# xxayt/MGSV

Measured on AMD Instinct MI355X. Metric: video-music pairs/s fwd+bwd at B=64 (full training step); sub-objects: retrieval sim-matrix GB/s, eval forward pairs/s, higher is better.
Workload: dtype bf16; 1 GPU; BASELINE.json configs[2]: B=64/GPU, T_v=30, T_a=512, D=512, train mode (dropout on), f32 master weights + Adam, f32 gradient accumulation; global_batch=64, launch=tape

## Files before the change

### include/made_hip.h

```cpp
#ifndef MADE_HIP_H
#define MADE_HIP_H

#include <stdint.h>

#ifdef __cplusplus
extern "C" {
#endif

#define MADE_ABI_VERSION 8

enum MadeDtype { MADE_F32 = 0, MADE_BF16 = 1 };

enum MadeAct {
    MADE_ACT_NONE = 0,
    MADE_ACT_RELU = 1,
    MADE_ACT_GELU = 2,
    MADE_ACT_QUICKGELU = 3,
    MADE_ACT_SIGMOID = 4
};

enum MadeGate {
    MADE_GATE_NONE = 0,
    MADE_GATE_RELU_OUT = 1,
    MADE_GATE_GELU_Z = 2,
// ... 438 lines not shown
                        float* save_mean, float* save_rstd, void* y, int32_t y_dtype, int64_t ldy,
                        int64_t B, int64_t T, int64_t F, void* stream);
int made_posbn_relu_bwd(const void* x, int32_t x_dtype, int64_t ldx, const void* y, int32_t y_dtype, int64_t ldy,
                        const void* dy, int32_t dy_dtype, int64_t lddy, const float* weight, const float* save_mean,
                        const float* save_rstd, int32_t batch_stats, void* dx, int32_t dx_dtype, int64_t lddx,
                        float* dweight, float* dbias, int64_t B, int64_t T, int64_t F, void* stream);

int made_set_criterion_bwd(const float* pred_logits, const float* pred_spans, const float* targets,
                           const int64_t* pred_idx, const int64_t* tgt_idx, const int32_t* count,
                           const float* proj_queries, const float* vid_sum, const float* empty_weight,
                           int64_t n_layers, int64_t B, int64_t Q, int64_t G, int64_t Dc, int32_t fg_label,
                           float temperature, const float* weights, const float* upstream,
                           float* d_logits, float* d_spans, int64_t ld_out, int32_t through_sigmoid,
                           float* d_proj_queries, float* d_vid_sum, void* stream);

#define MADE_ADAM_MAX_GROUPS 4
#define MADE_ADAM_NORM_BLOCKS 1024
typedef struct MadeAdamGroup { int64_t begin, end; float lr; float max_norm; } MadeAdamGroup;
int made_adam_step(float* param, const float* grad, float* exp_avg, float* exp_avg_sq, int64_t n,
                   const MadeAdamGroup* groups, int32_t n_groups, float beta1, float beta2, float eps, int64_t step,
                   float grad_scale, float* norm_ws, void* stream);

typedef struct MadeAdamDeviceState { int64_t step; float lr[MADE_ADAM_MAX_GROUPS]; float bc1, bc2_sqrt; } MadeAdamDeviceState;
int made_adam_step_device(float* param, const float* grad, float* exp_avg, float* exp_avg_sq, int64_t n,
                          const MadeAdamGroup* groups, int32_t n_groups, float beta1, float beta2, float eps,
                          MadeAdamDeviceState* state_device, int32_t advance_state, float grad_scale, float* norm_ws, void* stream);

typedef struct MadeRepackDesc {
    const float* src; void* w; void* wt;
    int64_t rows, cols, wt_ld, tile_begin;
// ... 85 lines not shown
```

### mgsv_amd/_lib.py

```python
from __future__ import annotations

import ctypes as C
import os

_HERE = os.path.dirname(os.path.abspath(__file__))


def variant_env(name: str, default: str = "") -> str:
    if os.environ.get("MADE_DEBUG_VARIANTS", "0") in ("", "0"):
        return default
    return os.environ.get(name, default)


LIB_PATH = os.environ.get("MADE_LIB_PATH") or os.path.join(_HERE, "libmade_hip.so")
ABI_VERSION = 8

F32, BF16 = 0, 1
ACT_NONE, ACT_RELU, ACT_GELU, ACT_QUICKGELU, ACT_SIGMOID = 0, 1, 2, 3, 4
GATE_NONE, GATE_RELU_OUT, GATE_GELU_Z, GATE_QUICKGELU_Z, GATE_SIGMOID_OUT = 0, 1, 2, 3, 4

vp, i64, i32, f32 = C.c_void_p, C.c_int64, C.c_int32, C.c_float


class MadeDropout(C.Structure):
# ... 214 lines not shown
    "made_pool_bwd": (C.c_int, [vp, vp, vp, vp, i32, i64, i64, vp, i32, i64, i64, vp, i32, i64, i64, i64, i64, i64, f32, vp]),
    "made_l2norm_bwd": (C.c_int, [vp, i32, i64, vp, i64, i64, vp, i64, i32, vp, i32, i64, i64, i64, f32, vp]),
    "made_clip_loss_bwd": (C.c_int, [vp, i64, i64, vp, f32, vp, vp, vp, vp, i32, vp, vp, vp]),
    "made_xpool_tail_bwd": (C.c_int, [vp, i32, i64, vp, vp, vp, i64, vp, i64, vp, i32, i64, vp, C.POINTER(MadeDropout),
                                      vp, vp, vp, i64, vp, i64, f32, i64, i64, i64, f32, vp]),
    "made_softmax_bwd": (C.c_int, [vp, i64, vp, i64, vp, i64, vp, f32, C.POINTER(MadeDropout), vp, vp, vp, i32, i64, i64,
                                   i64, i64, i64, i64, i64, vp]),
    "made_head_bias": (C.c_int, [vp, i32, i64, vp, vp, i64, i64, i64, vp]),
    "made_head_bias_bwd": (C.c_int, [vp, i32, i64, vp, vp, vp, vp, i64, i64, i64, vp]),
    "made_add3": (C.c_int, [vp, i32, vp, i32, vp, i32, vp, i32, i64, i64, vp]),
    "made_colsum": (C.c_int, [vp, i32, i64, i64, i64, vp, vp]),
    "made_posbn_relu_fwd": (C.c_int, [vp, i32, i64, vp, vp, vp, vp, C.c_float, C.c_float, i32, vp, vp, vp, i32, i64, i64, i64, i64, vp]),
    "made_posbn_relu_bwd": (C.c_int, [vp, i32, i64, vp, i32, i64, vp, i32, i64, vp, vp, vp, i32, vp, i32, i64, vp, vp, i64, i64, i64, vp]),
    "made_set_criterion_bwd": (C.c_int, [vp, vp, vp, vp, vp, vp, vp, vp, vp, i64, i64, i64, i64, i64, i32, f32, vp, vp,
                                         vp, vp, i64, i32, vp, vp, vp]),
    "made_adam_step": (C.c_int, [vp, vp, vp, vp, i64, C.POINTER(MadeAdamGroup), i32, f32, f32, f32, i64, f32, vp, vp]),
    "made_adam_step_device": (C.c_int, [vp, vp, vp, vp, i64, C.POINTER(MadeAdamGroup), i32, f32, f32, f32, vp, i32, f32, vp, vp]),
    "made_repack": (C.c_int, [vp, i32, i64, vp]),
    "made_row_groups": (C.c_int, [vp, i64, vp, vp]),
    "made_row_index": (C.c_int, [vp, i64, vp, vp, vp]),
    "made_linear_variant": (C.c_int, [C.POINTER(MadeLinearArgs)]),
    "made_row_affine": (C.c_int, [vp, i32, i64, vp, vp, i64, i32, vp, i32, i64, i64, i64, vp]),
    "made_gate_rows": (C.c_int, [vp, i32, i64, vp, i32, i64, i32, f32, vp, i64, i64, vp, i32, i64, vp, i64, i64, vp]),
    "made_xpool_fused": (C.c_int, [C.POINTER(MadeXpoolFusedArgs), vp]),
    "made_xpool_attention": (C.c_int, [C.POINTER(MadeXpoolAttnArgs), vp]),
    "made_xpool_sims": (C.c_int, [C.POINTER(MadeXpoolSimsArgs), vp]),
    "made_xpool_sims_ws_bytes": (C.c_int64, [i64, i64, i64]),
    "made_xpool_inbatch": (C.c_int, [C.POINTER(MadeXpoolInbatchArgs), vp]),
    "made_xpool_inbatch_ws_bytes": (C.c_int64, [i64, i64]),
    "made_batch_order": (C.c_int, [vp, i64, i64, vp, vp]),
# ... 60 lines not shown
```

### mgsv_amd/csrc/matcher.hip

```cpp
#include "common.h"
#pragma clang fp contract(off)

namespace {

constexpr int MAXN = 64;

__device__ __forceinline__ float giou_se(float s1, float e1, float s2, float e2) {
    float a1 = __fsub_rn(e1, s1), a2 = __fsub_rn(e2, s2);
    float inter = fmaxf(__fsub_rn(fminf(e1, e2), fmaxf(s1, s2)), 0.f);
    float uni = __fsub_rn(__fadd_rn(a1, a2), inter);
    float iou = __fdiv_rn(inter, uni);
    float enc = fmaxf(__fsub_rn(fmaxf(e1, e2), fminf(s1, s2)), 0.f);
    return __fsub_rn(iou, __fdiv_rn(__fsub_rn(enc, uni), enc));
}

__device__ __forceinline__ void cw_to_se(float c, float w, float& s, float& e) {
    float hw = __fmul_rn(0.5f, w);
    s = __fsub_rn(c, hw);
    e = __fadd_rn(c, hw);
}

__global__ __launch_bounds__(64) void hungarian_kernel(const float* logits, const float* spans, const float* targets,
                                                       int B, int Q, int G, int fg, float w_span, float w_giou, float w_class,
                                                       float* cost_ws, int cost_is_input, int64_t* out_pred, int64_t* out_tgt,
// ... 116 lines not shown
    v = wave_sum(v);
    __syncthreads();
    if ((threadIdx.x & 63) == 0) red[threadIdx.x >> 6] = v;
    __syncthreads();
    float t = (red[0] + red[1]) + (red[2] + red[3]);
    return t;
}

__device__ __forceinline__ int kth_kept(const float* tg, int G, int k) {
    int seen = 0;
    for (int g = 0; g < G; ++g)
        if (tg[2 * g + 1] != 0.f) { if (seen == k) return g; ++seen; }
    return 0;
}

__global__ __launch_bounds__(CRIT_THREADS) void criterion_kernel(const float* logits, const float* spans, const float* targets,
                                                                 const int64_t* pred_idx, const int64_t* tgt_idx, const int32_t* count,
                                                                 const float* proj_q, const float* vid_sum, const float* empty_w,
                                                                 int n_layers, int B, int Q, int G, int Dc, int fg, float temperature,
                                                                 const float* weights, float* losses, float* total) {
    __shared__ unsigned char matched[CRIT_MAX_BQ];
    __shared__ float lgt[CRIT_MAX_BQ];
    __shared__ float red[4];
    const int tid = threadIdx.x, lane = tid & 63, wave = tid >> 6;
    const int width = Q < G ? Q : G;
    const int bg = 1 - fg;
    {
        const int l = blockIdx.x;
        const float* lg = logits + (int64_t)l * B * Q * 2;
        const float* sp = spans + (int64_t)l * B * Q * 2;
        for (int i = tid; i < B * Q; i += CRIT_THREADS) matched[i] = 0;
        if (proj_q && vid_sum) {
            const bool vec = (Dc % 4 == 0) && (((uintptr_t)proj_q | (uintptr_t)vid_sum) % 16 == 0);
            for (int i = tid >> 2; i < B * Q; i += CRIT_THREADS / 4) {
                const int b = i / Q, part = tid & 3;
                const float* pq = proj_q + ((int64_t)l * B * Q + i) * Dc;
                const float* vs = vid_sum + (int64_t)b * Dc;
                float d = 0.f;
                if (vec) {
                    for (int k = part * 4; k < Dc; k += 16) {
                        const f32x4 x = *(const f32x4*)(pq + k), y = *(const f32x4*)(vs + k);
                        d += x[0] * y[0] + x[1] * y[1] + x[2] * y[2] + x[3] * y[3];
                    }
// ... 55 lines not shown
                csum += -pos / npos + (mx + logf(se));
            }
            contr = block_sum(csum, red) / (float)B;
        }
        if (tid == 0) {
            float ls = span_sum / (2.f * npairs);
            float lgi = giou_sum / npairs;
            float ll = label_sum / (float)(B * Q);
            float ce = 100.f - correct * (100.f / npairs);
            float* o = losses + l * 5;
            o[0] = ls; o[1] = lgi; o[2] = ll; o[3] = ce; o[4] = contr;
        }
    }
}

__global__ void criterion_total_kernel(const float* losses, const float* weights, int n_layers, float* total) {
    if (threadIdx.x != 0) return;
    float t = 0.f;
    for (int l = 0; l < n_layers; ++l) {
        const float* o = losses + l * 5;
        t += weights[0] * o[0] + weights[1] * o[1] + weights[2] * o[2] + weights[4] * o[4];
    }
    total[0] = t;
}

__global__ __launch_bounds__(CRIT_THREADS) void criterion_bwd_kernel(const float* logits, const float* spans, const float* targets,
                                                                     const int64_t* pred_idx, const int64_t* tgt_idx, const int32_t* count,
                                                                     const float* proj_q, const float* vid_sum, const float* empty_w,
                                                                     int B, int Q, int G, int Dc, int fg, float temperature,
                                                                     const float* weights, const float* upstream,
                                                                     float* dlogits, float* dspans, int ldo, int through_sigmoid,
                                                                     float* dproj_q, float* dvid_sum) {
    __shared__ unsigned char matched[CRIT_MAX_BQ];
    __shared__ float lgt[CRIT_MAX_BQ];
    __shared__ float red[4];
    const int tid = threadIdx.x, lane = tid & 63, wave = tid >> 6;
    const int width = Q < G ? Q : G;
    const int bg = 1 - fg;
    const int l = blockIdx.x;
    const int slice = blockIdx.y, nslice = gridDim.y;
    const float up = upstream ? upstream[0] : 1.f;
    const float* lg = logits + (int64_t)l * B * Q * 2;
    const float* sp = spans + (int64_t)l * B * Q * 2;
    float* dlg = dlogits + (int64_t)l * B * Q * ldo;
    float* dsp = dspans + (int64_t)l * B * Q * ldo;
    for (int i = tid; i < B * Q; i += CRIT_THREADS) {
        matched[i] = 0;
        if (slice == 0) { dsp[ldo * i] = 0.f; dsp[ldo * i + 1] = 0.f; }
    }
    __syncthreads();
    float npairs = 0.f;
    for (int i = tid; i < B * width; i += CRIT_THREADS) {
        int b = i / width, slot = i % width;
        if (slot < count[l * B + b]) npairs += 1.f;
    }
// ... 63 lines not shown
            for (int q = 0; q < Q; ++q) { mx = fmaxf(mx, lgt[b * Q + q]); npos += matched[b * Q + q] ? 1.f : 0.f; }
            float se = 0.f;
            for (int q = 0; q < Q; ++q) se += expf(lgt[b * Q + q] - mx);
            const float dl = wc * (expf(lgt[i] - mx) / se - (matched[i] ? 1.f / npos : 0.f));
            const float* pq = proj_q + ((int64_t)l * B * Q + i) * Dc;
            const float* vs = vid_sum + (int64_t)b * Dc;
            float* dpq = dproj_q + ((int64_t)l * B * Q + i) * Dc;
            for (int k = lane; k < Dc; k += 64) {
                dpq[k] = dl * vs[k];
                unsafeAtomicAdd(dvid_sum + (int64_t)b * Dc + k, dl * pq[k]);
            }
        }
    }
}

}

extern "C" int made_hungarian_match(const float* pred_logits, const float* pred_spans, const float* targets,
                                    int64_t NS, int64_t B, int64_t Q, int64_t G, int32_t fg_label,
                                    float w_span, float w_giou, float w_class,
                                    float* cost_ws, int32_t cost_is_input, int64_t* out_pred_idx, int64_t* out_tgt_idx,
                                    int32_t* out_count, int32_t* status, void* stream) {
    MADE_REQUIRE(pred_logits && pred_spans && targets && cost_ws && out_pred_idx && out_tgt_idx && out_count && status,
                 "made_hungarian_match: null pointer");
    MADE_REQUIRE(NS >= 0 && B > 0 && NS % B == 0, "made_hungarian_match: NS=%lld must be a multiple of B=%lld", (long long)NS, (long long)B);
    MADE_REQUIRE(fg_label == 0 || fg_label == 1, "made_hungarian_match: fg_label must be 0 or 1");
    MADE_UNSUPPORTED(Q >= 1 && G >= 1 && Q <= MAXN && G <= MAXN, "made_hungarian_match: Q=%lld, G=%lld must be in [1,%d]",
                     (long long)Q, (long long)G, MAXN);
    if (NS == 0) return MADE_OK;
    hipLaunchKernelGGL(hungarian_kernel, dim3((unsigned)NS), dim3(64), 0, (hipStream_t)stream, pred_logits, pred_spans, targets,
// ... 26 lines not shown
                                      int64_t n_layers, int64_t B, int64_t Q, int64_t G, int64_t Dc, int32_t fg_label,
                                      float temperature, const float* weights, const float* upstream,
                                      float* d_logits, float* d_spans, int64_t ld_out, int32_t through_sigmoid,
                                      float* d_proj_queries, float* d_vid_sum, void* stream) {
    MADE_REQUIRE(pred_logits && pred_spans && targets && pred_idx && tgt_idx && count && empty_weight && weights && d_logits && d_spans,
                 "made_set_criterion_bwd: null pointer");
    MADE_REQUIRE(n_layers >= 1 && B >= 1 && Q >= 1 && G >= 1, "made_set_criterion_bwd: bad dims");
    MADE_UNSUPPORTED(n_layers <= 65535 && B * Q <= CRIT_MAX_BQ, "made_set_criterion_bwd: B*Q=%lld exceeds %d", (long long)(B * Q), CRIT_MAX_BQ);
    const unsigned nslice = (proj_queries && vid_sum && d_proj_queries && d_vid_sum) ? (unsigned)(B < 16 ? B : 16) : 1u;
    hipLaunchKernelGGL(criterion_bwd_kernel, dim3((unsigned)n_layers, nslice), dim3(CRIT_THREADS), 0, (hipStream_t)stream, pred_logits, pred_spans,
                       targets, pred_idx, tgt_idx, count, proj_queries, vid_sum, empty_weight, (int)B, (int)Q, (int)G, (int)Dc,
                       (int)fg_label, temperature, weights, upstream, d_logits, d_spans, (int)(ld_out > 0 ? ld_out : 2), (int)through_sigmoid,
                       d_proj_queries, d_vid_sum);
    return made_check_launch("made_set_criterion_bwd");
}
```

### mgsv_amd/ops.py

```python
from __future__ import annotations

import ctypes as C
import math
from dataclasses import dataclass
from typing import Optional, Sequence

import torch

from . import _lib, tape as _tape
from ._lib import (ACT_GELU, ACT_NONE, ACT_QUICKGELU, ACT_RELU, ACT_SIGMOID, BF16, F32,
                   MadeAttnArgs, MadeDecStageArgs, MadeFinishArgs, MadeLinearArgs, MadeLinearSeg, MadeWideAttnArgs, check, lib)

Tensor = torch.Tensor


def dt_of(t: Tensor) -> int:
    if t.dtype == torch.float32:
        return F32
    if t.dtype == torch.bfloat16:
        return BF16
    raise TypeError(f"unsupported dtype {t.dtype}")


def torch_dtype(code: int):
# ... 662 lines not shown
    _timed("xpool_inbatch", 4.0 * Nv * Nm * S * D, float(2 * (K.numel() + U.numel()) + out.element_size() * Nv * Nm * D + 2 * Q.numel()),
           lambda: check(lib().made_xpool_inbatch(C.byref(a), _stream()), "made_xpool_inbatch"), desc)
    return out


def clip_loss(sims: Tensor, logit_scale: Tensor, loss_out: Tensor, weight: float = 1.0, accumulate: bool = False,
              row_exclude: Optional[Tensor] = None) -> Tensor:
    assert sims.dim() == 2 and sims.shape[0] == sims.shape[1] and sims.stride(1) == 1 and sims.dtype == torch.float32
    assert row_exclude is None or (row_exclude.shape == sims.shape and row_exclude.is_contiguous())
    check(lib().made_clip_loss(_p(sims), sims.stride(0), sims.shape[0], _p(logit_scale), weight, 1 if accumulate else 0,
                               _p(loss_out), _p(_f32(row_exclude, "row_exclude")), _stream()), "made_clip_loss")
    return loss_out


def hungarian_match(pred_logits: Tensor, pred_spans: Tensor, targets: Tensor, fg_label: int,
                    w_span: float = 10.0, w_giou: float = 1.0, w_class: float = 4.0, cost_in: Optional[Tensor] = None):
    NS, Q, _ = pred_logits.shape
    B, G, _ = targets.shape
    dev = pred_logits.device
    width = min(Q, G)
    if cost_in is not None:
        assert cost_in.shape == (NS, Q, G) and cost_in.dtype == torch.float32 and cost_in.is_contiguous()
        cost = cost_in
    else:
        cost = torch.empty((NS, Q, G), device=dev, dtype=torch.float32)
    pi = torch.empty((NS, width), device=dev, dtype=torch.int64)
    ti = torch.empty((NS, width), device=dev, dtype=torch.int64)
    cnt = torch.empty((NS,), device=dev, dtype=torch.int32)
    status = _tape.zero_(torch.empty((1,), device=dev, dtype=torch.int32))
    check(lib().made_hungarian_match(_p(_f32(pred_logits, "pred_logits")), _p(_f32(pred_spans, "pred_spans")),
                                     _p(_f32(targets, "targets")), NS, B, Q, G, fg_label, w_span, w_giou, w_class,
                                     _p(cost), 1 if cost_in is not None else 0, _p(pi), _p(ti), _p(cnt), _p(status), _stream()), "made_hungarian_match")
    return pi, ti, cnt, status, cost


def set_criterion(pred_logits: Tensor, pred_spans: Tensor, targets: Tensor, pred_idx: Tensor, tgt_idx: Tensor,
                  count: Tensor, proj_queries: Optional[Tensor], vid_sum: Optional[Tensor], empty_weight: Tensor,
                  fg_label: int, weights: Tensor, temperature: float = 0.07):
    nl, B, Q, _ = pred_logits.shape
    G = targets.shape[1]
    Dc = proj_queries.shape[-1] if proj_queries is not None else 0
    dev = pred_logits.device
    losses = torch.empty((nl, 5), device=dev, dtype=torch.float32)
    total = torch.empty((1,), device=dev, dtype=torch.float32)
# ... 97 lines not shown
```

### mgsv_amd/ops_train.py

```python
from __future__ import annotations

import ctypes as C
from typing import Optional, Tuple

import torch

from . import _lib
from ._lib import BF16, F32, MadeAttnBwdArgs, MadeDropout, MadeGemmTNArgs, MadeGemmTNGroup, check, lib
from .ops import _f32, _p, _stream, _timed, dt_of, set_drop

Tensor = torch.Tensor
Pair = Tuple[int, int]


_TN_SLAB_US = 1.3


def _tn_splits(tiles: int, nslab: int, gathered: bool, cap: int) -> int:
    if _lib.variant_env("MADE_TN_SPLIT_MODEL", "1") == "0":
        sp = max(8, (512 // max(tiles, 1)) // 8 * 8) if cap == 64 and tiles < 64 else max(1, 2048 // max(tiles, 1))
        while (nslab + sp - 1) // sp > 64:
            sp += 8
        return min(sp, max(1, nslab))
    live = max(1, (nslab * 9) // 16 if gathered else nslab)
# ... 365 lines not shown
    return out


def posbn_relu_bwd(x: Tensor, y: Tensor, dy: Tensor, weight: Tensor, save_mean: Tensor, save_rstd: Tensor, batch_stats: bool, dx: Tensor,
                   dweight: Optional[Tensor], dbias: Optional[Tensor]) -> Tensor:
    B, T, F = x.shape
    for t in (x, y, dy, dx):
        assert t.is_contiguous() and tuple(t.shape) == (B, T, F)
    check(lib().made_posbn_relu_bwd(_p(x), dt_of(x), F, _p(y), dt_of(y), F, _p(dy), dt_of(dy), F, _p(_f32(weight, "weight")),
                                    _p(_f32(save_mean, "save_mean")), _p(_f32(save_rstd, "save_rstd")), int(bool(batch_stats)),
                                    _p(dx), dt_of(dx), F, _p(_f32(dweight, "dweight")), _p(_f32(dbias, "dbias")), B, T, F, _stream()),
          "made_posbn_relu_bwd")
    return dx


def set_criterion_bwd(logits: Tensor, spans: Tensor, targets: Tensor, pi: Tensor, ti: Tensor, cnt: Tensor, pq: Optional[Tensor],
                      vid_sum: Optional[Tensor], empty_weight: Tensor, fg: int, weights: Tensor, upstream: Optional[Tensor],
                      d_logits: Tensor, d_spans: Tensor, d_pq: Optional[Tensor], d_vid_sum: Optional[Tensor],
                      temperature: float = 0.07, ld_out: int = 2, through_sigmoid: bool = False) -> None:
    nd, B, Q, _ = logits.shape
    G = targets.shape[1]
    Dc = pq.shape[-1] if pq is not None else 0
    check(lib().made_set_criterion_bwd(_p(logits), _p(spans), _p(targets), _p(pi), _p(ti), _p(cnt), _p(pq), _p(vid_sum),
                                       _p(empty_weight), nd, B, Q, G, Dc, fg, temperature, _p(weights), _p(upstream),
                                       _p(d_logits), _p(d_spans), ld_out, int(through_sigmoid), _p(d_pq), _p(d_vid_sum), _stream()),
          "made_set_criterion_bwd")
```

### mgsv_amd/trainer.py

```python
from __future__ import annotations

import math
import os
from typing import Dict, List, Optional, Tuple

import numpy as np
import torch

from . import _lib, dropout as dr, ops, ops_train as tr, tape as _tape
from .config import MadeConfig
from .engine import MadeEngine
from .ops import Seg, round_up

Tensor = torch.Tensor
XA = "video_guided_to_music_pooling_cross_transformer"


HEAD_PAD = 64


class MadeTrainer(MadeEngine):
    def __init__(self, cfg: MadeConfig, state_dict: Dict[str, object], device="cuda:0", dtype: str = "f32"):
        if dtype == "f32x3":
            raise ValueError('dtype "f32x3" (split-bf16 products) is an inference mode: it meets the forward\'s 1e-4 gate, its gradients do not meet '
# ... 283 lines not shown
                                                        float(betas[1]), float(eps), device_state.data_ptr(), 0 if part == "rest" else 1,
                                                        float(grad_scale), ws.data_ptr(), torch.cuda.current_stream().cuda_stream),
                       "made_adam_step_device")
            self.repack(part)
            return
        _lib.check(_lib.lib().made_adam_step(self.flat_param.data_ptr(), self.flat_grad.data_ptr(), self.exp_avg.data_ptr(),
                                             self.exp_avg_sq.data_ptr(), self.flat_param.numel(), groups, 3, float(betas[0]), float(betas[1]),
                                             float(eps), self.opt_step, float(grad_scale), ws.data_ptr(),
                                             torch.cuda.current_stream().cuda_stream), "made_adam_step")
        self.repack(part)

    def train_step(self, frame_feats, segment_feats, frame_masks, segment_masks, spans_target, seed: int, lrs=(1e-4, 1e-4, 1e-4),
                   max_grad_norm: float = 1.0, w_ret: Optional[Tensor] = None, w_loc: Optional[Tensor] = None, dist=None,
                   music_ids=None, v_duration: Optional[Tensor] = None) -> Dict[str, Tensor]:
        self._zero_grad_in_forward = True
        try:
            out = self.forward_train(frame_feats, segment_feats, frame_masks, segment_masks, spans_target, seed=seed, music_ids=music_ids,
                                     v_duration=v_duration)
        finally:
            self._zero_grad_in_forward = False
        scale = 1.0
        if dist is not None and dist.get_world_size() > 1:
            cut = self.group_ranges[0][1]
            works = []
            self.backward(w_ret, w_loc, grad_sync=lambda: works.append(dist.all_reduce(self.flat_grad[cut:], async_op=True)))
            works.append(dist.all_reduce(self.flat_grad[:cut], async_op=True))
            for w in works:
                w.wait()
            scale = 1.0 / dist.get_world_size()
        elif self._early_opt_ok():
            self.backward(w_ret, w_loc, early_opt=lambda: self.optimizer_step(*lrs, max_grad_norm=max_grad_norm, part="early"))
            self.optimizer_step(*lrs, max_grad_norm=max_grad_norm, part="rest")
            return out
        else:
            self.backward(w_ret, w_loc)
# ... 267 lines not shown
                                  drop=self._drop(f"dec.{l}" + ".sa_attn", pd))
                ta = ops.linear(tw[d + ".att"], P[p + ".sa.out.w"], P[p + ".sa.out.b"], R=tgt, out=tw[d + ".t_a"], drop=self._drop(f"dec.{l}" + ".drop1", pd))
                t1 = tw[d + ".t1"]
                ops.layernorm_add(ta, P[p + ".ln1.g"], P[p + ".ln1.b"], qp.expand(B * Q, D) if Q == 1 else qp.repeat(B, 1), t1, tw[d + ".t1q"])
                qc = ops.linear(tw[d + ".t1q"], Win[:D], bin_[:D], out=tw[d + ".qc"])
            qprime = GQ[:, 1, l]
            ops.linear(qc[:, :hd], Wt[:, D:D + hd], None, M=B * Q, N=D, K=hd, batch=H, a_z_stride=hd, w_z_stride=hd,
                       segs=[Seg(out=qprime, ldo=D, rows_per_batch=Q, out_batch_stride=qprime.stride(0), out_z_stride=Q * D)])

        dec_early = None
        side.wait_stream(cur)
        with torch.cuda.stream(side):
            if getattr(self, "_zero_grad_in_forward", False):
                _tape.zero_(self.flat_grad)
                self._grads_zeroed = True
            if (Q == 1 and not regression and c.moment_query_type != "xpool" and c.detr_enc_layers > 0
                    and _lib.variant_env("MADE_DEC_EARLY", "1") != "0"):
                dec_fill_tgt()
                dec_query_side(0)
                dec_early = torch.cuda.Event()
                dec_early.record(side)
            xmask = sm if c.fusion_mask == 1 else None
            if "music" in c.vmr_fusion:
                self._xpool_train(video, seg, xmask, ws, tw, B, Ta)
            if "video" in c.vmr_fusion and c.vmr_loss == "single":
                self._xpool_train(music, frame, fm if c.fusion_mask == 1 else None, ws, tw, B, Tv, key="xav", pre="y", sims_out=tw["sims_vp_t"])
                if "music" in c.vmr_fusion:
                    ws["sims_single"].add_(tw["sims_vp_t"].t())
                else:
                    ws["sims_single"].copy_(tw["sims_vp_t"].t())
                out["sims_video_pooling"] = tw["sims_vp_t"].t()
            ops.l2norm_rows(video, out_f32=tw["vn"]); ops.l2norm_rows(music, out_f32=tw["mn"])
# ... 145 lines not shown
        if c.contrastive_align_loss:
            ops.linear(hs2, P["proj_q.w"], P["proj_q.b"], out=ws["pq_raw"])
            pq = ws["pq"]
            pq2 = pq.view(nd * B * Q, -1)
            if c.audio_short_cut:
                mq = music if Q == 1 else music[:, None, :].expand(B, Q, D).contiguous()
                ops.l2norm_rows(ws["pq_raw"], out_f32=tw["pq_n0"])
                tr.add3(tw["pq_s1"], tw["pq_n0"], mq, b_mod=B * Q * D)
                ops.l2norm_rows(tw["pq_s1"], out_f32=pq2)
                if c.aux_loss and nd > 1:
                    n_aux = (nd - 1) * B * Q
                    tr.add3(tw["pq_s2"][:n_aux], pq2[:n_aux], mq, b_mod=B * Q * D)
                    ops.l2norm_rows(tw["pq_s2"][:n_aux], out_f32=pq2[:n_aux])
            else:
                ops.l2norm_rows(ws["pq_raw"], out_f32=pq2)
            self._frame_rows_linear(frame, P["proj_v.w"], P["proj_v.b"], ws["pv_raw"], B, Tv)
            pv = ws["pv"]
            ops.l2norm_rows(ws["pv_raw"], out_f32=pv.view(B * Tv, pq.shape[-1]))
            vid_sum = ops.masked_mean(pv, None, out=ws["vid_sum"])
            out.update(proj_queries=pq[-1], proj_vid_mem=pv, proj_queries_all=pq)
        tg = self._inputs[4]
        pi, ti, cnt, status, cost = ops.hungarian_match(logits.view(nd * B, Q, 2), spans.view(nd * B, Q, 2), tg, c.foreground_label)
        losses, total = ops.set_criterion(logits, spans, tg, pi, ti, cnt, pq, vid_sum, P["empty_weight"], c.foreground_label, P["crit_weights"])
        self._match = (pi, ti, cnt)
        out.update(matcher_pred_idx=pi.view(nd, B, -1), matcher_tgt_idx=ti.view(nd, B, -1), matcher_count=cnt.view(nd, B),
                   matcher_status=status, criterion_losses=losses, localization_loss=total)
        cur.wait_stream(side)
        return out

    def _opt_stream(self):
        st = getattr(self, "_opt_st", None)
        if st is None:
            st = self._opt_st = torch.cuda.Stream(device=self.device)
        return st

    def _dec_stage_chain(self) -> bool:
        c = self.cfg
        return (self.tc == torch.bfloat16 and c.num_moment_queries == 1 and c.D in (256, 512) and not c.detr_pre_norm
                and _lib.variant_env("MADE_DEC_STAGE", "1") != "0")

    def _encode_train(self, feats: Tensor, mask: Tensor, which: str, ws, tw, row_off: int) -> None:
        c, P = self.cfg, self.P
        if c.agg_module == "mlp":
            return self._encode_train_mlp(feats, mask, which, ws, tw, row_off)
        B, T, Kin = feats.shape
        D, Hh = c.D, c.SA_temporal_heads
        proj, mod, pe, depth, tag = (("vit_proj", "video_transformer", "pe_video", c.video_transformer_depth, "v") if which == "video"
                                     else ("ast_proj", "audio_transformer", "pe_audio", c.audio_transformer_depth, "a"))
        cls = bool(c.with_cls_token)
# ... 194 lines not shown
        D, L, Q, nd, ne, H = c.D, (Tv + Ta if concat else Ta), c.num_moment_queries, c.detr_dec_layers, c.detr_enc_layers, c.detr_nheads
        hd, HQ = D // H, H * Q
        pd = float(c.detr_dropout)
        inv_keep = 1.0 / (1.0 - pd) if (self.training_dropout and pd > 0) else 1.0
        fus, fus_mask = ws["fus"], ws["fus_mask"]
        fskip = fus_mask.view(-1)
        qskip = fus_mask
        regression = "regression" in c.mml_localization
        if regression:
            fskip = qskip = None
        rows = B * L
        if zero_grad and not getattr(self, "_grads_zeroed", False):
            _tape.zero_(self.flat_grad)
        self._grads_zeroed = False
        dvideo, dmusic = tw["dvideo"], tw["dmusic"]
        _tape.zero_(tw["dclip"])
        video, music = ws["video"], ws["music"]
        frame, seg_view = self._views
        cur, side = torch.cuda.current_stream(), self._side_stream()
        xq = c.moment_query_type == "xpool" and not regression
        side.wait_stream(cur)
        ret_done = None
        ret_gen = None
        if not xq:
            ret_main = _lib.variant_env("MADE_RET_BWD_MAIN", "0") == "1"
            ret_split = (_lib.variant_env("MADE_RET_SPLIT", "1") != "0" and not ret_main and not regression
                         and _lib.variant_env("MADE_RET_HANDOFF", "") == "" and _lib.variant_env("MADE_RET_HANDOFF_REV", "") == "")
            with torch.cuda.stream(cur if ret_main else side):
                self._ret_main_stream = cur
                try:
                    self._ret_ck(0)
# ... 5 lines not shown
                        self._retrieval_bwd(ws, tw, g_ret, B, Ta, sm)
                    on_main = torch.cuda.current_stream() == cur
                finally:
                    self._ret_main_stream = None
                if ret_gen is None:
                    ret_done = torch.cuda.Event()
                    ret_done.record(cur if on_main else side)

        if regression:
            dmem, dtgt0 = self._regression_bwd(ws, tw, g_loc, B, L), None
        else:
            logits, spans = ws["logits"], ws["spans"]
            pi, ti, cnt = self._match
            pq = ws["pq"] if c.contrastive_align_loss else None
            vid_sum = ws["vid_sum"] if c.contrastive_align_loss else None
            tr.set_criterion_bwd(logits, spans, tg, pi, ti, cnt, pq, vid_sum, P["empty_weight"], c.foreground_label, P["crit_weights"], g_loc,
                                 tw["dlog"], tw["dsp"], tw["dpq"] if pq is not None else None, tw["dvid_sum"] if pq is not None else None,
                                 ld_out=HEAD_PAD, through_sigmoid=True)
            hs2 = ws["hs"].view(nd * B * Q, D)
            dhs = tw["dhs"]
            dlog, dsp = tw["dlog"], tw["dsp"]
            if self.tc != torch.float32:
                tr.add3(tw["dlogsp_c"], tw["dlogsp"])
                dlog, dsp = tw["dlog_c"], tw["dsp_c"]
            heads_dw: list = []
            heads_dw.append(lambda: tr.gemm_tn(dlog[:, :2], hs2, G["class_embed.w"], accumulate=True, colsum=G["class_embed.b"]))
            ops.linear(dlog, P["class_embed.wt"], None, out=dhs)
            n_span = 1 if c.predict_center == 1 else 2
            heads_dw.append(lambda: tr.gemm_tn(dsp[:, :n_span], tw["h2"], G["span_embed.2.w"], accumulate=True, colsum=G["span_embed.2.b"]))
            dz2 = ops.linear(dsp, P["span_embed.2.wt"], None, out=tw["hg1"], gate=_lib.GATE_RELU_OUT, G=tw["h2"])
            dz1 = self._lin_bwd(dz2, tw["h1"], "span_embed.1", dx_out=tw["hg2"], gate=_lib.GATE_RELU_OUT, G=tw["h1"], later=heads_dw)
            self._lin_bwd(dz1, hs2, "span_embed.0", dx_out=dhs, R=dhs, later=heads_dw)
            if c.contrastive_align_loss:
                Dc = pq.shape[-1]
                dn = tw["dpq"]
                if c.audio_short_cut:
                    if c.aux_loss and nd > 1:
                        n_aux = (nd - 1) * B * Q
                        ds2 = tw["dpq_s2"][:n_aux]
                        tr.l2norm_bwd(tw["pq_s2"][:n_aux], dn[:n_aux], dx=ds2)
                        dmusic.add_(ds2.view(nd - 1, B, Q, D).sum((0, 2)))
                        dn[:n_aux].copy_(ds2)
                    tr.l2norm_bwd(tw["pq_s1"], dn, dx=tw["dpq_s"])
                    dmusic.add_(tw["dpq_s"].view(nd, B, Q, D).sum((0, 2)))
                    dn = tw["dpq_s"]
                tr.l2norm_bwd(ws["pq_raw"], dn, dx_alt=tw["dpq_raw"])
                self._lin_bwd(tw["dpq_raw"], hs2, "proj_q", dx_out=dhs, R=dhs, later=heads_dw)
                tr.l2norm_bwd(ws["pv_raw"], tw["dvid_sum"], dx_alt=tw["dpv_raw"], dy_rows_per=Tv)
                heads_dw.append(lambda: tr.gemm_tn(tw["dpv_raw"][:Tv], frame[0], G["proj_v.w"], accumulate=True, colsum=G["proj_v.b"], batch=(B, 1),
                                                   a_zs=(Tv * Dc, 0), b_zs=(frame.stride(0), 0), colsum_zs=(0, 0)))
                ops.linear(tw["dpv_raw"], P["proj_v.wt"], None, out=tw["dframe_x"])

            qp = P["query_embed"]
            mem3, mempos3 = tw["mem"].view(B, L, D), tw["mempos"].view(B, L, D)
            Lp = tw["PdS"].shape[-1]
            GQ, PdS = tw["GQ"], tw["PdS"]
            ca_scale = 1.0 / math.sqrt(hd)
            st = tw["dstack"]
            dtgt = None
            stage = self._dec_stage_chain()
            pre = bool(c.detr_pre_norm)
            S_all = tw["dS_S"]
            if not stage:
                ops.linear(GQ[0, 1].reshape(nd * HQ, D), mempos3[0], None, M=nd * HQ, N=L, K=D, batch=B, a_z_stride=GQ.stride(0), w_z_stride=L * D,
                           segs=[Seg(out=S_all, ldo=Lp, rows_per_batch=HQ, out_batch_stride=B * HQ * Lp, out_z_stride=HQ * Lp)])
            n_split_b = int(_lib.variant_env("MADE_WIDE_NSPLIT", "0")) or max(1, min(8, 256 // max(B, 1)))
# ... 635 lines not shown
        S = _lib.MadeAdamDeviceState
        assert C.sizeof(S) % 8 == 0 and S.step.offset == 0 and S.lr.offset % 4 == 0
        self.adam_state = torch.zeros(C.sizeof(S) // 8, device=dev, dtype=torch.int64)
        lr0 = S.lr.offset // 4
        self._lr_view = self.adam_state.view(torch.float32)[lr0:lr0 + 3]
        self._lrs: Optional[tuple] = None
        ex = t.same_music_exclusion(music_ids)
        self.exclusion = ex.clone() if ex is not None else None
        scale = 1.0 / self.dist.get_world_size() if self.dist is not None else 1.0
        i = self.inputs

        early = self.dist is None and t._early_opt_ok()

        def fwd_bwd():
            t._zero_grad_in_forward = True
            try:
                out = t.forward_train(i["frame_feats"], i["segment_feats"], i["frame_masks"], i["segment_masks"], i["spans_target"], seed=0,
                                      v_duration=self.v_duration)
            finally:
                t._zero_grad_in_forward = False
            if early:
                t.backward(None, None, early_opt=lambda: t.optimizer_step(0.0, 0.0, 0.0, max_grad_norm=max_grad_norm, grad_scale=scale,
                                                                           device_state=self.adam_state, part="early"))
            else:
                t.backward(None, None)
            return out

        def opt():
            t.optimizer_step(0.0, 0.0, 0.0, max_grad_norm=max_grad_norm, grad_scale=scale, device_state=self.adam_state,
                             part="rest" if early else None)

        keep = [x.clone() for x in (t.flat_param, t.exp_avg, t.exp_avg_sq)]
        keep_buf = {k: v.clone() for k, v in t.buffers.items()}
        keep_step, keep_gen = t.opt_step, t.generation
        t._seed_dev, t._static_exclusion = self.seed_dev, self.exclusion
# ... 10 lines not shown
            for k, v in keep_buf.items():
                t.buffers[k].copy_(v)
            t.opt_step, t.generation = keep_step, keep_gen
            t.repack()
            self.adam_state[0] = keep_step
            torch.cuda.synchronize()
            self.graphs = []
            if mode == "tape":
                keep2 = [x.clone() for x in (t.flat_param, t.exp_avg, t.exp_avg_sq)]
                if self.dist is not None:
                    dist_, works = self.dist, []
                    cut = t.group_ranges[0][1]

                    def fwd_bwd():
                        t._zero_grad_in_forward = True
                        try:
                            out = t.forward_train(i["frame_feats"], i["segment_feats"], i["frame_masks"], i["segment_masks"], i["spans_target"], seed=0,
                                                  v_duration=self.v_duration)
                        finally:
                            t._zero_grad_in_forward = False
                        t.backward(None, None, grad_sync=lambda: _tape.callback(lambda: works.append(dist_.all_reduce(t.flat_grad[cut:], async_op=True))))
                        _tape.callback(lambda: works.append(dist_.all_reduce(t.flat_grad[:cut], async_op=True)))

                        def wait_all():
                            for w in works:
                                w.wait()
                            works.clear()
                        _tape.callback(wait_all)
                        return out
                try:
                    with _tape.LaunchTape.record(check=os.environ.get("MADE_TAPE_CHECK", "1") != "0") as tp:
                        self.out = fwd_bwd(); opt()
                    torch.cuda.synchronize()
                    self.tape = tp
                    tw_ = int(_lib.variant_env("MADE_TAPE_INTERLEAVE", "2"))
# ... 98 lines not shown
```

Measured before the change: 13880 pairs/s.

## Fuse set-criterion loss and backward into one forward-time kernel launch

Adds a fused criterion kernel whose grid runs gradient slices and per-layer loss blocks together, with a ticket atomic so the last loss block computes the total. In the captured training step it runs during forward and replaces the separate loss, total and backward launches. It also moves proj_v forward earlier, zeroes dclip in forward, and defers the proj_v l2norm and linear backward into the heads_dw list so they can overlap. The cost is a persistent ticket buffer and more coupling between forward and backward state.

```diff
diff --git a/include/made_hip.h b/include/made_hip.h
--- a/include/made_hip.h
+++ b/include/made_hip.h
@@ -476,6 +476,15 @@
                            float* d_logits, float* d_spans, int64_t ld_out, int32_t through_sigmoid,
                            float* d_proj_queries, float* d_vid_sum, void* stream);
 
+int made_set_criterion_fused(const float* pred_logits, const float* pred_spans, const float* targets,
+                             const int64_t* pred_idx, const int64_t* tgt_idx, const int32_t* count,
+                             const float* proj_queries, const float* vid_sum, const float* empty_weight,
+                             int64_t n_layers, int64_t B, int64_t Q, int64_t G, int64_t Dc, int32_t fg_label,
+                             float temperature, const float* weights, const float* upstream,
+                             float* losses, float* total, uint32_t* ticket,
+                             float* d_logits, float* d_spans, int64_t ld_out, int32_t through_sigmoid,
+                             float* d_proj_queries, float* d_vid_sum, void* stream);
+
 #define MADE_ADAM_MAX_GROUPS 4
 #define MADE_ADAM_NORM_BLOCKS 1024
 typedef struct MadeAdamGroup { int64_t begin, end; float lr; float max_norm; } MadeAdamGroup;
diff --git a/mgsv_amd/_lib.py b/mgsv_amd/_lib.py
--- a/mgsv_amd/_lib.py
+++ b/mgsv_amd/_lib.py
@@ -252,6 +252,8 @@
     "made_posbn_relu_bwd": (C.c_int, [vp, i32, i64, vp, i32, i64, vp, i32, i64, vp, vp, vp, i32, vp, i32, i64, vp, vp, i64, i64, i64, vp]),
     "made_set_criterion_bwd": (C.c_int, [vp, vp, vp, vp, vp, vp, vp, vp, vp, i64, i64, i64, i64, i64, i32, f32, vp, vp,
                                          vp, vp, i64, i32, vp, vp, vp]),
+    "made_set_criterion_fused": (C.c_int, [vp, vp, vp, vp, vp, vp, vp, vp, vp, i64, i64, i64, i64, i64, i32, f32, vp, vp,
+                                           vp, vp, vp, vp, vp, i64, i32, vp, vp, vp]),
     "made_adam_step": (C.c_int, [vp, vp, vp, vp, i64, C.POINTER(MadeAdamGroup), i32, f32, f32, f32, i64, f32, vp, vp]),
     "made_adam_step_device": (C.c_int, [vp, vp, vp, vp, i64, C.POINTER(MadeAdamGroup), i32, f32, f32, f32, vp, i32, f32, vp, vp]),
     "made_repack": (C.c_int, [vp, i32, i64, vp]),
diff --git a/mgsv_amd/csrc/matcher.hip b/mgsv_amd/csrc/matcher.hip
--- a/mgsv_amd/csrc/matcher.hip
+++ b/mgsv_amd/csrc/matcher.hip
@@ -154,19 +154,15 @@
     return 0;
 }
 
-__global__ __launch_bounds__(CRIT_THREADS) void criterion_kernel(const float* logits, const float* spans, const float* targets,
-                                                                 const int64_t* pred_idx, const int64_t* tgt_idx, const int32_t* count,
-                                                                 const float* proj_q, const float* vid_sum, const float* empty_w,
-                                                                 int n_layers, int B, int Q, int G, int Dc, int fg, float temperature,
-                                                                 const float* weights, float* losses, float* total) {
-    __shared__ unsigned char matched[CRIT_MAX_BQ];
-    __shared__ float lgt[CRIT_MAX_BQ];
-    __shared__ float red[4];
-    const int tid = threadIdx.x, lane = tid & 63, wave = tid >> 6;
+__device__ __forceinline__ void criterion_layer_losses(const int l, unsigned char* matched, float* lgt, float* red,
+                                                       const float* logits, const float* spans, const float* targets,
+                                                       const int64_t* pred_idx, const int64_t* tgt_idx, const int32_t* count,
+                                                       const float* proj_q, const float* vid_sum, const float* empty_w,
+                                                       int B, int Q, int G, int Dc, int fg, float temperature, float* losses) {
+    const int tid = threadIdx.x;
     const int width = Q < G ? Q : G;
     const int bg = 1 - fg;
     {
-        const int l = blockIdx.x;
         const float* lg = logits + (int64_t)l * B * Q * 2;
         const float* sp = spans + (int64_t)l * B * Q * 2;
         for (int i = tid; i < B * Q; i += CRIT_THREADS) matched[i] = 0;
@@ -252,31 +248,43 @@
     }
 }
 
-__global__ void criterion_total_kernel(const float* losses, const float* weights, int n_layers, float* total) {
-    if (threadIdx.x != 0) return;
+__global__ __launch_bounds__(CRIT_THREADS) void criterion_kernel(const float* logits, const float* spans, const float* targets,
+                                                                 const int64_t* pred_idx, const int64_t* tgt_idx, const int32_t* count,
+                                                                 const float* proj_q, const float* vid_sum, const float* empty_w,
+                                                                 int n_layers, int B, int Q, int G, int Dc, int fg, float temperature,
+                                                                 const float* weights, float* losses, float* total) {
+    __shared__ unsigned char matched[CRIT_MAX_BQ];
+    __shared__ float lgt[CRIT_MAX_BQ];
+    __shared__ float red[4];
+    criterion_layer_losses(blockIdx.x, matched, lgt, red, logits, spans, targets, pred_idx, tgt_idx, count, proj_q, vid_sum, empty_w,
+                           B, Q, G, Dc, fg, temperature, losses);
+}
+
+__device__ __forceinline__ float criterion_total(const float* losses, const float* weights, int n_layers) {
     float t = 0.f;
     for (int l = 0; l < n_layers; ++l) {
         const float* o = losses + l * 5;
         t += weights[0] * o[0] + weights[1] * o[1] + weights[2] * o[2] + weights[4] * o[4];
     }
-    total[0] = t;
-}
-
-__global__ __launch_bounds__(CRIT_THREADS) void criterion_bwd_kernel(const float* logits, const float* spans, const float* targets,
-                                                                     const int64_t* pred_idx, const int64_t* tgt_idx, const int32_t* count,
-                                                                     const float* proj_q, const float* vid_sum, const float* empty_w,
-                                                                     int B, int Q, int G, int Dc, int fg, float temperature,
-                                                                     const float* weights, const float* upstream,
-                                                                     float* dlogits, float* dspans, int ldo, int through_sigmoid,
-                                                                     float* dproj_q, float* dvid_sum) {
-    __shared__ unsigned char matched[CRIT_MAX_BQ];
-    __shared__ float lgt[CRIT_MAX_BQ];
-    __shared__ float red[4];
+    return t;
+}
+
+__global__ void criterion_total_kernel(const float* losses, const float* weights, int n_layers, float* total) {
+    if (threadIdx.x != 0) return;
+    total[0] = criterion_total(losses, weights, n_layers);
+}
+
+__device__ __forceinline__ void criterion_layer_grads(const int l, const int slice, const int nslice, unsigned char* matched, float* lgt,
+                                                      float* red, const float* logits, const float* spans, const float* targets,
+                                                      const int64_t* pred_idx, const int64_t* tgt_idx, const int32_t* count,
+                                                      const float* proj_q, const float* vid_sum, const float* empty_w,
+                                                      int B, int Q, int G, int Dc, int fg, float temperature,
+                                                      const float* weights, const float* upstream,
+                                                      float* dlogits, float* dspans, int ldo, int through_sigmoid,
+                                                      float* dproj_q, float* dvid_sum) {
     const int tid = threadIdx.x, lane = tid & 63, wave = tid >> 6;
     const int width = Q < G ? Q : G;
     const int bg = 1 - fg;
-    const int l = blockIdx.x;
-    const int slice = blockIdx.y, nslice = gridDim.y;
     const float up = upstream ? upstream[0] : 1.f;
     const float* lg = logits + (int64_t)l * B * Q * 2;
     const float* sp = spans + (int64_t)l * B * Q * 2;
@@ -370,6 +378,54 @@
     }
 }
 
+__global__ __launch_bounds__(CRIT_THREADS) void criterion_bwd_kernel(const float* logits, const float* spans, const float* targets,
+                                                                     const int64_t* pred_idx, const int64_t* tgt_idx, const int32_t* count,
+                                                                     const float* proj_q, const float* vid_sum, const float* empty_w,
+                                                                     int B, int Q, int G, int Dc, int fg, float temperature,
+                                                                     const float* weights, const float* upstream,
+                                                                     float* dlogits, float* dspans, int ldo, int through_sigmoid,
+                                                                     float* dproj_q, float* dvid_sum) {
+    __shared__ unsigned char matched[CRIT_MAX_BQ];
+    __shared__ float lgt[CRIT_MAX_BQ];
+    __shared__ float red[4];
+    criterion_layer_grads(blockIdx.x, blockIdx.y, gridDim.y, matched, lgt, red, logits, spans, targets, pred_idx, tgt_idx, count, proj_q,
+                          vid_sum, empty_w, B, Q, G, Dc, fg, temperature, weights, upstream, dlogits, dspans, ldo, through_sigmoid,
+                          dproj_q, dvid_sum);
+}
+
+__global__ __launch_bounds__(CRIT_THREADS) void criterion_fused_kernel(const float* logits, const float* spans, const float* targets,
+                                                                       const int64_t* pred_idx, const int64_t* tgt_idx, const int32_t* count,
+                                                                       const float* proj_q, const float* vid_sum, const float* empty_w,
+                                                                       int n_layers, int nslice, int B, int Q, int G, int Dc, int fg,
+                                                                       float temperature, const float* weights, const float* upstream,
+                                                                       float* losses, float* total, unsigned* ticket,
+                                                                       float* dlogits, float* dspans, int ldo, int through_sigmoid,
+                                                                       float* dproj_q, float* dvid_sum) {
+    __shared__ unsigned char matched[CRIT_MAX_BQ];
+    __shared__ float lgt[CRIT_MAX_BQ];
+    __shared__ float red[4];
+    const int l = blockIdx.x;
+    if ((int)blockIdx.y < nslice) {
+        criterion_layer_grads(l, blockIdx.y, nslice, matched, lgt, red, logits, spans, targets, pred_idx, tgt_idx, count, proj_q, vid_sum,
+                              empty_w, B, Q, G, Dc, fg, temperature, weights, upstream, dlogits, dspans, ldo, through_sigmoid, dproj_q,
+                              dvid_sum);
+        return;
+    }
+    criterion_layer_losses(l, matched, lgt, red, logits, spans, targets, pred_idx, tgt_idx, count, proj_q, vid_sum, empty_w, B, Q, G, Dc,
+                           fg, temperature, losses);
+    if (threadIdx.x == 0) {
+        __builtin_amdgcn_fence(__ATOMIC_RELEASE, "agent");
+        asm volatile("s_waitcnt vmcnt(0)" ::: "memory");
+        const unsigned drawn = __hip_atomic_fetch_add(ticket, 1u, __ATOMIC_RELAXED, __HIP_MEMORY_SCOPE_AGENT);
+        if (drawn == (unsigned)n_layers - 1u) {
+            __builtin_amdgcn_fence(__ATOMIC_ACQUIRE, "agent");
+            asm volatile("s_waitcnt vmcnt(0)" ::: "memory");
+            total[0] = criterion_total(losses, weights, n_layers);
+            __hip_atomic_store(ticket, 0u, __ATOMIC_RELAXED, __HIP_MEMORY_SCOPE_AGENT);
+        }
+    }
+}
+
 }
 
 extern "C" int made_hungarian_match(const float* pred_logits, const float* pred_spans, const float* targets,
@@ -426,3 +482,25 @@
                        d_proj_queries, d_vid_sum);
     return made_check_launch("made_set_criterion_bwd");
 }
+
+extern "C" int made_set_criterion_fused(const float* pred_logits, const float* pred_spans, const float* targets,
+                                        const int64_t* pred_idx, const int64_t* tgt_idx, const int32_t* count,
+                                        const float* proj_queries, const float* vid_sum, const float* empty_weight,
+                                        int64_t n_layers, int64_t B, int64_t Q, int64_t G, int64_t Dc, int32_t fg_label,
+                                        float temperature, const float* weights, const float* upstream,
+                                        float* losses, float* total, uint32_t* ticket,
+                                        float* d_logits, float* d_spans, int64_t ld_out, int32_t through_sigmoid,
+                                        float* d_proj_queries, float* d_vid_sum, void* stream) {
+    MADE_REQUIRE(pred_logits && pred_spans && targets && pred_idx && tgt_idx && count && empty_weight && weights && losses && total && ticket
+                 && d_logits && d_spans, "made_set_criterion_fused: null pointer");
+    MADE_REQUIRE(n_layers >= 1 && B >= 1 && Q >= 1 && G >= 1, "made_set_criterion_fused: bad dims");
+    MADE_UNSUPPORTED(n_layers <= 65535 && B * Q <= CRIT_MAX_BQ, "made_set_criterion_fused: B*Q=%lld exceeds %d", (long long)(B * Q), CRIT_MAX_BQ);
+    const bool contr = proj_queries && vid_sum;
+    MADE_REQUIRE(!contr || (d_proj_queries && d_vid_sum), "made_set_criterion_fused: proj_queries without d_proj_queries / d_vid_sum");
+    const unsigned nslice = contr ? (unsigned)(B < 16 ? B : 16) : 1u;
+    hipLaunchKernelGGL(criterion_fused_kernel, dim3((unsigned)n_layers, nslice + 1u), dim3(CRIT_THREADS), 0, (hipStream_t)stream, pred_logits,
+                       pred_spans, targets, pred_idx, tgt_idx, count, proj_queries, vid_sum, empty_weight, (int)n_layers, (int)nslice, (int)B,
+                       (int)Q, (int)G, (int)Dc, (int)fg_label, temperature, weights, upstream, losses, total, (unsigned*)ticket, d_logits,
+                       d_spans, (int)(ld_out > 0 ? ld_out : 2), (int)through_sigmoid, d_proj_queries, d_vid_sum);
+    return made_check_launch("made_set_criterion_fused");
+}
diff --git a/mgsv_amd/ops.py b/mgsv_amd/ops.py
--- a/mgsv_amd/ops.py
+++ b/mgsv_amd/ops.py
@@ -700,7 +700,8 @@
 
 
 def hungarian_match(pred_logits: Tensor, pred_spans: Tensor, targets: Tensor, fg_label: int,
-                    w_span: float = 10.0, w_giou: float = 1.0, w_class: float = 4.0, cost_in: Optional[Tensor] = None):
+                    w_span: float = 10.0, w_giou: float = 1.0, w_class: float = 4.0, cost_in: Optional[Tensor] = None,
+                    status: Optional[Tensor] = None):
     NS, Q, _ = pred_logits.shape
     B, G, _ = targets.shape
     dev = pred_logits.device
@@ -713,7 +714,9 @@
     pi = torch.empty((NS, width), device=dev, dtype=torch.int64)
     ti = torch.empty((NS, width), device=dev, dtype=torch.int64)
     cnt = torch.empty((NS,), device=dev, dtype=torch.int32)
-    status = _tape.zero_(torch.empty((1,), device=dev, dtype=torch.int32))
+    if status is None:
+        status = _tape.zero_(torch.empty((1,), device=dev, dtype=torch.int32))
+    assert status.dtype == torch.int32 and status.numel() == 1
     check(lib().made_hungarian_match(_p(_f32(pred_logits, "pred_logits")), _p(_f32(pred_spans, "pred_spans")),
                                      _p(_f32(targets, "targets")), NS, B, Q, G, fg_label, w_span, w_giou, w_class,
                                      _p(cost), 1 if cost_in is not None else 0, _p(pi), _p(ti), _p(cnt), _p(status), _stream()), "made_hungarian_match")
diff --git a/mgsv_amd/ops_train.py b/mgsv_amd/ops_train.py
--- a/mgsv_amd/ops_train.py
+++ b/mgsv_amd/ops_train.py
@@ -403,6 +403,22 @@
     return dx
 
 
+def set_criterion_fused(logits: Tensor, spans: Tensor, targets: Tensor, pi: Tensor, ti: Tensor, cnt: Tensor, pq: Optional[Tensor],
+                        vid_sum: Optional[Tensor], empty_weight: Tensor, fg: int, weights: Tensor, upstream: Optional[Tensor],
+                        losses: Tensor, total: Tensor, ticket: Tensor, d_logits: Tensor, d_spans: Tensor, d_pq: Optional[Tensor],
+                        d_vid_sum: Optional[Tensor], temperature: float = 0.07, ld_out: int = 2, through_sigmoid: bool = False) -> None:
+    nd, B, Q, _ = logits.shape
+    G = targets.shape[1]
+    Dc = pq.shape[-1] if pq is not None else 0
+    assert tuple(losses.shape) == (nd, 5) and losses.dtype == torch.float32 and losses.is_contiguous() and total.dtype == torch.float32
+    assert ticket.dtype == torch.int32 and ticket.numel() == 1
+    check(lib().made_set_criterion_fused(_p(_f32(logits, "logits")), _p(_f32(spans, "spans")), _p(_f32(targets, "targets")), _p(pi), _p(ti),
+                                         _p(cnt), _p(_f32(pq, "proj_queries")), _p(_f32(vid_sum, "vid_sum")), _p(_f32(empty_weight, "empty_weight")),
+                                         nd, B, Q, G, Dc, fg, temperature, _p(_f32(weights, "weights")), _p(upstream), _p(losses), _p(total),
+                                         _p(ticket), _p(d_logits), _p(d_spans), ld_out, int(through_sigmoid), _p(d_pq), _p(d_vid_sum), _stream()),
+          "made_set_criterion_fused")
+
+
 def set_criterion_bwd(logits: Tensor, spans: Tensor, targets: Tensor, pi: Tensor, ti: Tensor, cnt: Tensor, pq: Optional[Tensor],
                       vid_sum: Optional[Tensor], empty_weight: Tensor, fg: int, weights: Tensor, upstream: Optional[Tensor],
                       d_logits: Tensor, d_spans: Tensor, d_pq: Optional[Tensor], d_vid_sum: Optional[Tensor],
diff --git a/mgsv_amd/trainer.py b/mgsv_amd/trainer.py
--- a/mgsv_amd/trainer.py
+++ b/mgsv_amd/trainer.py
@@ -321,11 +321,13 @@
                    max_grad_norm: float = 1.0, w_ret: Optional[Tensor] = None, w_loc: Optional[Tensor] = None, dist=None,
                    music_ids=None, v_duration: Optional[Tensor] = None) -> Dict[str, Tensor]:
         self._zero_grad_in_forward = True
+        self._step_w_loc = (w_loc,)
         try:
             out = self.forward_train(frame_feats, segment_feats, frame_masks, segment_masks, spans_target, seed=seed, music_ids=music_ids,
                                      v_duration=v_duration)
         finally:
             self._zero_grad_in_forward = False
+            self._step_w_loc = None
         scale = 1.0
         if dist is not None and dist.get_world_size() > 1:
             cut = self.group_ranges[0][1]
@@ -623,8 +625,17 @@
             if getattr(self, "_zero_grad_in_forward", False):
                 _tape.zero_(self.flat_grad)
                 self._grads_zeroed = True
+            self._dclip_zeroed = False
+            pv_early, status_pre = False, None
             if (Q == 1 and not regression and c.moment_query_type != "xpool" and c.detr_enc_layers > 0
                     and _lib.variant_env("MADE_DEC_EARLY", "1") != "0"):
+                if c.contrastive_align_loss:
+                    self._proj_v_fwd(ws, frame, B, Tv)
+                    pv_early = True
+                if getattr(self, "_step_w_loc", None) is not None and self._heads_fused():
+                    _tape.zero_(tw["dclip"])
+                    self._dclip_zeroed = True
+                    status_pre = _tape.zero_(torch.empty((1,), device=self.device, dtype=torch.int32))
                 dec_fill_tgt()
                 dec_query_side(0)
                 dec_early = torch.cuda.Event()
@@ -800,25 +811,56 @@
                     ops.l2norm_rows(tw["pq_s2"][:n_aux], out_f32=pq2[:n_aux])
             else:
                 ops.l2norm_rows(ws["pq_raw"], out_f32=pq2)
-            self._frame_rows_linear(frame, P["proj_v.w"], P["proj_v.b"], ws["pv_raw"], B, Tv)
-            pv = ws["pv"]
-            ops.l2norm_rows(ws["pv_raw"], out_f32=pv.view(B * Tv, pq.shape[-1]))
-            vid_sum = ops.masked_mean(pv, None, out=ws["vid_sum"])
+            if not pv_early:
+                self._proj_v_fwd(ws, frame, B, Tv)
+            pv, vid_sum = ws["pv"], ws["vid_sum"]
             out.update(proj_queries=pq[-1], proj_vid_mem=pv, proj_queries_all=pq)
         tg = self._inputs[4]
-        pi, ti, cnt, status, cost = ops.hungarian_match(logits.view(nd * B, Q, 2), spans.view(nd * B, Q, 2), tg, c.foreground_label)
-        losses, total = ops.set_criterion(logits, spans, tg, pi, ti, cnt, pq, vid_sum, P["empty_weight"], c.foreground_label, P["crit_weights"])
+        pi, ti, cnt, status, cost = ops.hungarian_match(logits.view(nd * B, Q, 2), spans.view(nd * B, Q, 2), tg, c.foreground_label,
+                                                        status=status_pre)
+        self._crit_bwd_done = False
+        if getattr(self, "_step_w_loc", None) is not None and self._heads_fused():
+            if not self._dclip_zeroed:
+                _tape.zero_(tw["dclip"])
+                self._dclip_zeroed = True
+            losses = torch.empty((nd, 5), device=self.device, dtype=torch.float32)
+            total = torch.empty((1,), device=self.device, dtype=torch.float32)
+            tr.set_criterion_fused(logits, spans, tg, pi, ti, cnt, pq, vid_sum, P["empty_weight"], c.foreground_label, P["crit_weights"],
+                                   self._step_w_loc[0], losses, total, self._crit_ticket(), tw["dlog"], tw["dsp"],
+                                   tw["dpq"] if pq is not None else None, tw["dvid_sum"] if pq is not None else None,
+                                   ld_out=HEAD_PAD, through_sigmoid=True)
+            self._crit_bwd_done = True
+        else:
+            losses, total = ops.set_criterion(logits, spans, tg, pi, ti, cnt, pq, vid_sum, P["empty_weight"], c.foreground_label, P["crit_weights"])
         self._match = (pi, ti, cnt)
         out.update(matcher_pred_idx=pi.view(nd, B, -1), matcher_tgt_idx=ti.view(nd, B, -1), matcher_count=cnt.view(nd, B),
                    matcher_status=status, criterion_losses=losses, localization_loss=total)
         cur.wait_stream(side)
         return out
 
+    def _proj_v_fwd(self, ws, frame: Tensor, B: int, Tv: int) -> None:
+        P = self.P
+        self._frame_rows_linear(frame, P["proj_v.w"], P["proj_v.b"], ws["pv_raw"], B, Tv)
+        pv = ws["pv"]
+        ops.l2norm_rows(ws["pv_raw"], out_f32=pv.view(B * Tv, pv.shape[-1]))
+        ops.masked_mean(pv, None, out=ws["vid_sum"])
+
+    def _crit_ticket(self) -> Tensor:
+        t = getattr(self, "_crit_tk", None)
+        if t is None:
+            t = self._crit_tk = torch.zeros(1, device=self.device, dtype=torch.int32)
+        return t
+
     def _opt_stream(self):
         st = getattr(self, "_opt_st", None)
         if st is None:
             st = self._opt_st = torch.cuda.Stream(device=self.device)
         return st
+
+    def _heads_fused(self) -> bool:
+        c = self.cfg
+        return (self.tc == torch.bfloat16 and c.D in (256, 512) and c.predict_center == 0 and not c.audio_short_cut and not c.moment_loss
+                and "regression" not in c.mml_localization and _lib.variant_env("MADE_HEADS_FUSED", "1") != "0")
 
     def _dec_stage_chain(self) -> bool:
         c = self.cfg
@@ -1043,7 +1085,9 @@
             _tape.zero_(self.flat_grad)
         self._grads_zeroed = False
         dvideo, dmusic = tw["dvideo"], tw["dmusic"]
-        _tape.zero_(tw["dclip"])
+        if not getattr(self, "_dclip_zeroed", False):
+            _tape.zero_(tw["dclip"])
+        self._dclip_zeroed = False
         video, music = ws["video"], ws["music"]
         frame, seg_view = self._views
         cur, side = torch.cuda.current_stream(), self._side_stream()
@@ -1079,9 +1123,12 @@
             pi, ti, cnt = self._match
             pq = ws["pq"] if c.contrastive_align_loss else None
             vid_sum = ws["vid_sum"] if c.contrastive_align_loss else None
-            tr.set_criterion_bwd(logits, spans, tg, pi, ti, cnt, pq, vid_sum, P["empty_weight"], c.foreground_label, P["crit_weights"], g_loc,
-                                 tw["dlog"], tw["dsp"], tw["dpq"] if pq is not None else None, tw["dvid_sum"] if pq is not None else None,
-                                 ld_out=HEAD_PAD, through_sigmoid=True)
+            if getattr(self, "_crit_bwd_done", False):
+                self._crit_bwd_done = False
+            else:
+                tr.set_criterion_bwd(logits, spans, tg, pi, ti, cnt, pq, vid_sum, P["empty_weight"], c.foreground_label, P["crit_weights"], g_loc,
+                                     tw["dlog"], tw["dsp"], tw["dpq"] if pq is not None else None, tw["dvid_sum"] if pq is not None else None,
+                                     ld_out=HEAD_PAD, through_sigmoid=True)
             hs2 = ws["hs"].view(nd * B * Q, D)
             dhs = tw["dhs"]
             dlog, dsp = tw["dlog"], tw["dsp"]
@@ -1111,10 +1158,10 @@
                     dn = tw["dpq_s"]
                 tr.l2norm_bwd(ws["pq_raw"], dn, dx_alt=tw["dpq_raw"])
                 self._lin_bwd(tw["dpq_raw"], hs2, "proj_q", dx_out=dhs, R=dhs, later=heads_dw)
-                tr.l2norm_bwd(ws["pv_raw"], tw["dvid_sum"], dx_alt=tw["dpv_raw"], dy_rows_per=Tv)
+                heads_dw.append(lambda: tr.l2norm_bwd(ws["pv_raw"], tw["dvid_sum"], dx_alt=tw["dpv_raw"], dy_rows_per=Tv))
+                heads_dw.append(lambda: ops.linear(tw["dpv_raw"], P["proj_v.wt"], None, out=tw["dframe_x"]))
                 heads_dw.append(lambda: tr.gemm_tn(tw["dpv_raw"][:Tv], frame[0], G["proj_v.w"], accumulate=True, colsum=G["proj_v.b"], batch=(B, 1),
                                                    a_zs=(Tv * Dc, 0), b_zs=(frame.stride(0), 0), colsum_zs=(0, 0)))
-                ops.linear(tw["dpv_raw"], P["proj_v.wt"], None, out=tw["dframe_x"])
 
             qp = P["query_embed"]
             mem3, mempos3 = tw["mem"].view(B, L, D), tw["mempos"].view(B, L, D)
@@ -1780,11 +1827,13 @@
 
         def fwd_bwd():
             t._zero_grad_in_forward = True
+            t._step_w_loc = (None,)
             try:
                 out = t.forward_train(i["frame_feats"], i["segment_feats"], i["frame_masks"], i["segment_masks"], i["spans_target"], seed=0,
                                       v_duration=self.v_duration)
             finally:
                 t._zero_grad_in_forward = False
+                t._step_w_loc = None
             if early:
                 t.backward(None, None, early_opt=lambda: t.optimizer_step(0.0, 0.0, 0.0, max_grad_norm=max_grad_norm, grad_scale=scale,
                                                                            device_state=self.adam_state, part="early"))
@@ -1825,11 +1874,13 @@
 
                     def fwd_bwd():
                         t._zero_grad_in_forward = True
+                        t._step_w_loc = (None,)
                         try:
                             out = t.forward_train(i["frame_feats"], i["segment_feats"], i["frame_masks"], i["segment_masks"], i["spans_target"], seed=0,
                                                   v_duration=self.v_duration)
                         finally:
                             t._zero_grad_in_forward = False
+                            t._step_w_loc = None
                         t.backward(None, None, grad_sync=lambda: _tape.callback(lambda: works.append(dist_.all_reduce(t.flat_grad[cut:], async_op=True))))
                         _tape.callback(lambda: works.append(dist_.all_reduce(t.flat_grad[:cut], async_op=True)))
 
```

Measured after the change: 13980 pairs/s (median of 6 runs). Within noise of the previous version (+0.8%).
